# daac-tools/daachorse

Hardware: AMD Instinct MI355X
Metric: haystack GB/s scanned (find_overlapping_iter(..).count(), 100k-pattern bytewise automaton) (higher is better)
Workload: dtype u8/u32 integer

## Files before the change

### daachorse_amd/_build.py

```python
import os
import shutil
import subprocess

_HERE = os.path.dirname(os.path.abspath(__file__))
CSRC = os.path.join(_HERE, "csrc")
LIB_DIR = os.path.join(_HERE, "lib")
LIB_PATH = os.path.join(LIB_DIR, "libdaachorse_amd.so")

SOURCES = ["pma.cpp", "repack.cpp", "gram.cpp", "gram2.cpp", "gram4.cpp", "gram2w.cpp", "pfx.cpp", "builder.cpp", "charwise.cpp", "charwise_builder.cpp", "api_upload.hip", "api_scan.hip", "api_select.hip", "api_iter.hip", "api_options.hip", "scan_kernels.hip",
           "gram_kernels.hip", "gram2_kernels.hip", "gram4_kernels.hip", "pfx_kernels.hip", "emit3_kernels.hip", "find3_kernels.hip", "left3_kernels.hip", "gram2w_kernels.hip", "restart_kernels.hip", "charwise_kernels.hip", "synth.hip",
           "api_batch.hip", "batch_kernels.hip", "batch_hist_kernels.hip", "api_hist.hip", "hist_kernels.hip", "api_replace.hip", "replace_kernels.hip", "api_tokenize.hip", "tokenize_kernels.hip", "api_unigram.hip", "unigram_kernels.hip", "api_bpe.hip", "bpe_kernels.hip", "api_split.hip", "split_kernels.hip", "api_wordpiece.hip", "wordpiece_kernels.hip", "api_normalize.hip", "normalize_kernels.hip"]
HEADERS = ["api_internal.hpp", "pma.hpp", "repack.hpp", "gram.hpp", "gram2.hpp", "gram4.hpp", "gram4_filter.hpp", "gram4_index.hpp", "gram4_mph.hpp", "gram2w.hpp", "pfx.hpp", "charwise.hpp", "build_common.hpp", "device_tables.hpp", "chain_scan.hpp", "scan_engines.hpp", "restart_tables.hpp", "char_tables.hpp", "batch.hpp", "hist.hpp", "replace.hpp", "tokenize.hpp", "unigram.hpp", "bpe.hpp", "split.hpp", "wordpiece.hpp", "normalize.hpp",
           os.path.join("..", "..", "include", "daachorse_amd.h"),
           os.path.join("..", "..", "include", "daac_synth.h")]


def _hipcc():
    for cand in (shutil.which("hipcc"), "/opt/rocm/bin/hipcc"):
        if cand and os.path.exists(cand):
            return cand
    raise RuntimeError("hipcc not found: the HIP extension cannot be built")


def source_hash():
    import hashlib
    h = hashlib.sha256()
    for f in SOURCES + HEADERS:
        path = os.path.join(CSRC, f)
        h.update(os.path.basename(f).encode() + b"\0")
        with open(path, "rb") as fh:
            h.update(fh.read())
    return h.hexdigest()


def needs_build():
    if not os.path.exists(LIB_PATH):
        return True
    t = os.path.getmtime(LIB_PATH)
    files = [os.path.join(CSRC, f) for f in SOURCES + HEADERS]
    return any(os.path.exists(f) and os.path.getmtime(f) > t for f in files)


def build(force=False, verbose=False):
    if not force and not needs_build():
        return LIB_PATH
# ... 27 lines not shown
```

### daachorse_amd/csrc/api_internal.hpp

```cpp
#pragma once
#include <hip/hip_runtime.h>

#include <algorithm>
#include <atomic>
#include <cassert>
#include <cstdlib>
#include <chrono>
#include <cstring>
#include <map>
#include <memory>
#include <condition_variable>
#include <deque>
#include <functional>
#include <mutex>
#include <string>
#include <thread>
#include <utility>
#include <vector>

#include "charwise.hpp"
#include "device_tables.hpp"
#include "gram.hpp"
#include "gram2.hpp"
#include "gram4.hpp"
#include "gram2w.hpp"
#include "pfx.hpp"
#include "pma.hpp"
#include "repack.hpp"

namespace daac {
const char *last_error_cstr();

#define DAAC_OPTIONS(X)                                                                                                                      \
    X(seg_bytes, 0, 0)                                                                                                         \
    X(lds_budget, 96 * 1024, 1)                                                                                                              \
    X(dense_depth, -1, 1)                                                                                                                    \
    X(rows_share_pct, 45, 1)                                                                                                                 \
    X(blocks_per_cu, 0, 0)                                                                                                     \
    X(threads, 1024, 0)                                                                                                                      \
    X(iter_window, 64ll << 20, 0)                  \
    X(max_result_bytes, 8ll << 30, 0)                                                                                                        \
    X(gram_lds_budget, 158 * 1024, 1)                                                                                                        \
    X(gram_region, 0, 0)                                          \
    X(gram_slab, 4096, 0)                                                                                                                    \
    X(gram_ppl, 0, 0)                                                                      \
    X(gram_dense, -1, 0)                                                                                      \
    X(gram_rank_in_lds, -1, 1)                                                                                \
    X(gram_version, 0, 0)                   \
    X(gram4_arith, 1, 0)                  \
    X(gram4_filter, 1, 0)                      \
    X(gram4_mph, 8, 1)                    \
    X(gram2_dpp, 1, 0)                                                  \
    X(find3, 1, 0)                                                                                         \
    X(pfx_probe, 16384, 0)                                                             \
    X(pfx, 1, 1)                                 \
    X(gram_tail, -1, 0)                         \
    X(gram2_rfull, 1, 0)                                                            \
    X(emit, 1, 0)                            \
    X(emit_rec_per_kib, 32, 0)                               \
    X(restart_bpc, 8, 0)                                                              \
    X(restart_chain, 1, 0)                      \
    X(chain_rounds, 24, 0)                                                                                                                   \
    X(overlap_micro, 1, 0)                \
    X(pool, 1, 0)                                                                 \
    X(pool_keep, 0, 0)                                                                    \
    X(left3, 1, 0)                        \
    X(select_emit, 1, 0)                                   \
    X(find3_window, 1ll << 30, 0)                                \
    X(workspace_keep, 8ll << 30, 0)                          \
    X(char_map_lds, 1, 1)                                         \
    X(char_row_lds, 1, 1)                                                                      \
    X(batch_piece, 4096, 0)                                              \
    X(batch_lane_max, 16384, 0)           \
    X(hist_lds_bins, 16384, 0)            \
    X(batch_hist_wave_max, 2048, 0)                  \
    X(batch_hist_sort_max, 16384, 0)      \
    X(bpe_doc_max, 4096, 0)
// ... 387 lines not shown
```

### daachorse_amd/csrc/api_scan.hip

```cpp
#include "api_internal.hpp"

static daac_status scan_count_impl(daac_pma *pma, int mode, int engine, const uint8_t *hay, size_t len, size_t begin, int hay_is_device,
                                   void *stream_, uint64_t *count, uint64_t *checksum, uint64_t *result_dev, bool want_checksum);

namespace {

__global__ void repack8_kernel(const uint4 *in, uint2 *out, unsigned long long n, unsigned long long base, uint32_t end_bits) {
    for (unsigned long long i = static_cast<unsigned long long>(blockIdx.x) * blockDim.x + threadIdx.x; i < n; i += static_cast<unsigned long long>(gridDim.x) * blockDim.x) {
        const uint4 t = in[i];
        const unsigned long long end = (static_cast<unsigned long long>(t.y) << 32) | t.x;
        out[i] = uint2{t.w, static_cast<uint32_t>(end - base) | (t.z << end_bits)};
    }
}
__global__ void repack16_kernel(const daac_match *in, uint4 *out, unsigned long long n) {
    for (unsigned long long i = static_cast<unsigned long long>(blockIdx.x) * blockDim.x + threadIdx.x; i < n; i += static_cast<unsigned long long>(gridDim.x) * blockDim.x) {
        const daac_match m = in[i];
        out[i] = uint4{static_cast<uint32_t>(m.end), static_cast<uint32_t>(m.end >> 32), static_cast<uint32_t>(m.end - m.start), m.value};
    }
}

__global__ void shard_subtract_kernel(unsigned long long *r, const unsigned long long *h, unsigned long long from32) {
    r[0] -= h[0];
    r[1] -= h[1];
    r[2] -= h[2];
    r[2] += (r[1] & 0xffffffffull) * from32;
}

__global__ void shard_fixup_kernel(unsigned long long *r, unsigned long long begin32, unsigned long long c, unsigned long long s1,
                                   unsigned long long s2) {
    r[2] += (r[1] & 0xffffffffull) * begin32 + s2;
    r[1] += s1;
    r[0] += c;
}
// ... 341 lines not shown
        if (!want_checksum && t->gram4_ok && (gv == 4 || gv == 0 || (gv == 2 && !t->gram2.exact_ok)) && gram4_shape(t, cp)) {
            cp.kernel = CountKernel::gram4; cp.threads = cp.g4.threads; cp.lds_bytes = cp.g4.lds_bytes; cp.wq_entry = sizeof(uint4);
            return cp;
        }
        if (gv == 4 && !want_checksum)
            return refuse("gram_version = 4: the gram4 tables are not there for this automaton (or do not fit the LDS with the launch shape asked for)", CountKernel::gram4);
        if (!t->gram2.exact_ok) return refuse("GRAM second table set: `.count()` runs on the gram4 kernel (gram_version 0 or 4); the count + checksum kernel needs tables this dictionary has no room for", CountKernel::gram2);
        cp.kernel = CountKernel::gram2; cp.lds_bytes = gram2_lds_bytes(t->gram2, want_checksum);
    } else if (gram && g1_can) {
        cp.kernel = CountKernel::gram; cp.lds_bytes = t->gram.lds_bytes; cp.ppl = !t->gram.has_short && OPT(gram_ppl) != 16 ? 32 : 16;
        cp.n_deep = t->gram.n_deep; cp.C = t->gram.C; cp.K = t->gram.K;
    } else if (gram) {
        cp.kernel = CountKernel::gram2w; cp.threads = 1024; cp.lds_bytes = want_checksum ? t->gramw.lds_exact : t->gramw.lds_count;
        cp.n_deep = t->gramw.n_deep; cp.C = t->gramw.C; cp.K = 2;
    } else if (pfx) {
        cp.kernel = CountKernel::pfx; cp.region[0] = 65536; cp.region[1] = 262144;
        cp.threads = t->pfx.threads; cp.lds_bytes = t->pfx.lds_bytes; cp.wq_entry = sizeof(uint4);
    } else {
        cp.charwise = pma->charwise; cp.tier = on_tier(pma, t, mode, engine);
    }
    return cp;
}

std::pair<int, int> count_ids(const DeviceTables *t, const CountPlan &cp) {
    switch (cp.kernel) {
    case CountKernel::gram4: return {DAAC_ENGINE_GRAM, DAAC_KERNEL_GRAM_COUNT};
    case CountKernel::gram: case CountKernel::gram2: return {DAAC_ENGINE_GRAM, DAAC_KERNEL_GRAM_EXACT};
    case CountKernel::gram2w: return {DAAC_ENGINE_GRAM, DAAC_KERNEL_GRAM_WIDE};
    case CountKernel::pfx: return {DAAC_ENGINE_PFX, DAAC_KERNEL_PFX};
    default: return {cp.tier ? DAAC_ENGINE_TIERED : DAAC_ENGINE_DARRAY, micro_walker(t, cp.charwise, cp.tier) ? DAAC_KERNEL_MICRO : DAAC_KERNEL_SEGMENT};
    }
}

static std::string count_kernel_name(const CountPlan &cp) {
    static const char *const family[] = {"gram4", "gram", "gram2", "gram2w", "pfx"};
    if (cp.kernel == CountKernel::walkers) return cp.charwise ? "charwise" : cp.tier ? "tiered" : "darray";
    if (cp.kernel != CountKernel::gram4) return family[static_cast<int>(cp.kernel)];
    return "gram4 ppl=" + std::to_string(cp.ppl) + " dir=" + std::to_string(cp.g4.dir) + " waves=" + std::to_string(cp.g4.threads / 64) + " arith=" +
           std::to_string(cp.g4.arith) + " filter=" + std::to_string(cp.g4.filter) + " mph=" + std::to_string(cp.g4.mph) + " tail=" + (OPT(gram_tail) < 0 ? std::string("auto") : std::to_string(OPT(gram_tail) > 0 ? 1 : 0));
}

}
}

extern "C" {

static daac_status scan_count_impl(daac_pma *pma, int mode, int engine, const uint8_t *hay, size_t len, size_t begin, int hay_is_device,
                                   void *stream_, uint64_t *count, uint64_t *checksum, uint64_t *result_dev, bool want_checksum) {
    PmaScope scope_(pma);
    if (!pma || (len && !hay) || (!result_dev && (!count || (want_checksum && !checksum))) || begin > len) {
        set_error("bad argument");
        return DAAC_ERR_INVALID_ARGUMENT;
    }
    hipStream_t stream = static_cast<hipStream_t>(stream_);
    DeviceTables *t = nullptr;
    dbg_mark("count: entry");
    daac_status st = check_mode_kind(pma, mode);
    if (st != DAAC_OK) return st;
    if ((st = get_tables(pma, &t)) != DAAC_OK) return st;
    CountPlan cp = resolve_count(pma, t, mode, engine, want_checksum, len - begin);
    if (cp.probe && hay_is_device && !result_dev && len - begin >= (32ull << 20) && t->pfx_probe_word) {
        unsigned int *pin = pinned_words();
        unsigned int got = 0;
        unsigned int *tmp = const_cast<unsigned int *>(t->pfx_probe_word);
        HIP_TRY(launch_pfx_probe(t->pfx, hay + begin, len - begin, tmp, stream));
        HIP_TRY(hipMemcpyAsync(pin ? pin : &got, tmp, 4, hipMemcpyDeviceToHost, stream));
        HIP_TRY(hipStreamSynchronize(stream));
        if (pin) got = *pin;
        t->pfx_dense.store(got > static_cast<unsigned int>(std::max<int64_t>(0, OPT(pfx_probe))) ? 1 : 0);
        cp = resolve_count(pma, t, mode, engine, want_checksum, len - begin);
    }
    if (cp.st != DAAC_OK) { set_error(cp.err); return cp.st; }
    Plan pl;
    bool heads = false;
    if ((st = make_plan(pma, t, mode, cp.kernel != CountKernel::walkers ? DAAC_ENGINE_AUTO : engine, begin, len, pl, heads)) != DAAC_OK) return st;
    if (pl.a.nseg == 0 && begin == 0) pl.a.nseg = 1;
    void *staged = nullptr;
    const uint8_t *dev_hay = hay;
    if (!hay_is_device && len) {
        const uint64_t from = begin > pl.a.halo ? begin - pl.a.halo : 0;
        if ((st = stage_window(hay, from, len, stream, &staged, &dev_hay)) != DAAC_OK) return st;
    }
    std::unique_ptr<void, void (*)(void *)> g1(staged, [](void *p) { if (p) (void)hipFree(p); });
    pl.a.hay = dev_hay;
    unsigned long long *d_res = reinterpret_cast<unsigned long long *>(result_dev);
    DevBuf own;
    if (!d_res) { HIP_TRY(own.alloc(3 * sizeof(unsigned long long), stream)); d_res = static_cast<unsigned long long *>(own.p); }
    pl.a.result = d_res;
    bool find3_served = false;
    unsigned long long find3_sums[3] = {0, 0, 0};
    dbg_mark("count: plan made");
    if (!pma->charwise && engine == DAAC_ENGINE_AUTO && !pma->root_has_output() && len != begin &&
        ((mode == DAAC_FIND && pma->host.is_standard()) || (mode == DAAC_LEFTMOST_FIND && !pma->host.is_standard()))) {
        if ((st = find_count3(pma, t, dev_hay, begin, len, stream, d_res, want_checksum, mode == DAAC_LEFTMOST_FIND, find3_sums, &find3_served)) != DAAC_OK) return st;
    }
    dbg_mark("count: find3 back");
    ChainBuffers chain_buffers;
    if (!find3_served && pl.a.nseg != 0 && (st = chain_resolve(pma, t, pl, stream, chain_buffers)) != DAAC_OK) return st;
    if (!find3_served) HIP_TRY(hipMemsetAsync(d_res, 0, 3 * sizeof(unsigned long long), stream));
    void *flagbuf = nullptr;
    if (pl.leftmost && pma->root_has_output()) {
        HIP_TRY(hipMalloc(&flagbuf, sizeof(unsigned long long)));
        HIP_TRY(hipMemsetAsync(flagbuf, 0, sizeof(unsigned long long), stream));
        pl.a.flags = static_cast<unsigned long long *>(flagbuf);
    }
    std::unique_ptr<void, void (*)(void *)> g3(flagbuf, [](void *p) { if (p) (void)hipFree(p); });
    if (!find3_served) g_last_engine = count_ids(t, cp).first;
    g_last_kernel = find3_served ? "find3" : count_kernel_name(cp);
    if (find3_served) {
    } else if (cp.kernel != CountKernel::walkers && len != begin) {
        const uint64_t from = begin - std::min<uint64_t>(begin, pl.a.halo);
        const uint8_t *sub = dev_hay + from;
        GramArgs ga{};
        ga.lead = static_cast<uint32_t>(reinterpret_cast<uintptr_t>(sub) & 15u);
        ga.hay_al = sub - ga.lead;
        ga.vlen = ga.lead + static_cast<uint64_t>(len - from);
        uint64_t region = 2048;
        const int64_t region_opt = OPT(gram_region) > 0 ? OPT(gram_region) : static_cast<int64_t>(cp.region[(len - from) >= (1ull << 31)]);
        while (region * 2 <= static_cast<uint64_t>(std::max<int64_t>(2048, region_opt)) && region < (1ull << 30)) region *= 2;
        assert((region & (region - 1)) == 0 && region <= (1ull << 30));
        ga.ppl = cp.ppl;
        ga.region_bytes = region;
        ga.nregions = (ga.vlen + region - 1) / region;
        ga.result = d_res;
        const uint32_t threads = cp.threads, wpb = threads / 64;
        uint32_t bpc = static_cast<uint32_t>(OPT(blocks_per_cu));
        if (bpc == 0) bpc = std::max(1u, std::min(2048u / threads, (160u * 1024u) / cp.lds_bytes));
        const uint32_t blocks = static_cast<uint32_t>(
            std::max<uint64_t>(1, std::min<uint64_t>(static_cast<uint64_t>(t->num_cu) * bpc, (ga.nregions + wpb - 1) / wpb)));
        ga.wq_slab = static_cast<uint32_t>(std::max<int64_t>(64 * ga.ppl + 128 + 64, OPT(gram_slab)));
        ga.dense = OPT(gram_dense) >= 0 ? OPT(gram_dense) != 0 : cp.n_deep * 100 > cp.C * cp.C * cp.C * (cp.K == 3 ? cp.C : 1);
        const int64_t tail_opt = OPT(gram_tail);
        void *wq = nullptr;
        HIP_TRY(dev_malloc(&wq, static_cast<size_t>(blocks) * wpb * ga.wq_slab * cp.wq_entry, stream));
        ga.wq = static_cast<uint2 *>(wq);
        ga.sel_want = tail_opt < 0 ? ((len - begin) >= (1ull << 20) ? 2u : 0u) : tail_opt > 0 ? 1u : 0u;
        auto launch_count = [&](const GramArgs &g, uint32_t nblocks) -> hipError_t {
            switch (cp.kernel) {
            case CountKernel::gram4: return launch_gram4_scan(t->gram4, g, cp.g4, nblocks, stream);
            case CountKernel::gram: return launch_gram_scan(t->gram, g, nblocks, threads, stream);
            case CountKernel::gram2: return launch_gram2_scan(t->gram2, g, want_checksum, nblocks, threads, stream);
            case CountKernel::gram2w: return launch_gram2w_scan(t->gramw, g, want_checksum, nblocks, stream);
            case CountKernel::pfx: return launch_pfx_scan(t->pfx, g, want_checksum, nblocks, stream);
            default: return hipErrorInvalidValue;
            }
        };
        hipError_t le = launch_count(ga, blocks);
        DevBuf halo_res;
        if (le == hipSuccess && from != begin) {
            le = halo_res.alloc(3 * sizeof(unsigned long long), stream);
            if (le == hipSuccess) le = hipMemsetAsync(halo_res.p, 0, 3 * sizeof(unsigned long long), stream);
            GramArgs gh = ga;
            gh.vlen = ga.lead + (begin - from);
            gh.nregions = (gh.vlen + gh.region_bytes - 1) / gh.region_bytes;
            gh.result = static_cast<unsigned long long *>(halo_res.p);
            gh.sel_want = 0;
            if (le == hipSuccess) le = launch_count(gh, 1);
            if (le == hipSuccess) {
                hipLaunchKernelGGL(shard_subtract_kernel, dim3(1), dim3(1), 0, stream, d_res, static_cast<const unsigned long long *>(halo_res.p),
                                   static_cast<unsigned long long>(from & 0xffffffffull));
                le = hipGetLastError();
            }
        } else if (le == hipSuccess && from != 0) {
            hipLaunchKernelGGL(shard_fixup_kernel, dim3(1), dim3(1), 0, stream, d_res, static_cast<unsigned long long>(from & 0xffffffffull), 0ull, 0ull, 0ull);
            le = hipGetLastError();
        }
        dev_free(wq, stream);
        HIP_TRY(le);
    } else if (pl.a.nseg != 0) {
        HIP_TRY(launch(t, pl, 0, heads, stream));
    }
    unsigned long long flagv = 0;
    if (flagbuf) HIP_TRY(hipMemcpyAsync(&flagv, flagbuf, sizeof(flagv), hipMemcpyDeviceToHost, stream));
    if (result_dev && !count) {
        if (staged || flagbuf) HIP_TRY(hipStreamSynchronize(stream));
        return (flagv & 1ull) ? diverged() : DAAC_OK;
    }
    unsigned long long r[3];
    if (find3_served) {
        std::memcpy(r, find3_sums, sizeof(r));
    } else {
        HIP_TRY(hipMemcpyAsync(r, d_res, sizeof(r), hipMemcpyDeviceToHost, stream));
        HIP_TRY(hipStreamSynchronize(stream));
    }
    dbg_mark("count: result read");
    if (flagv & 1ull) return diverged();
    if (count) *count = r[0];
// ... 276 lines not shown
```

### daachorse_amd/csrc/device_tables.hpp

```cpp
#pragma once

#include <hip/hip_runtime.h>

#include <cstdint>

#include "../../include/daachorse_amd.h"
#include "gram4_mph.hpp"

namespace daac {

struct TierDev {
    const void *rows;
    const uint32_t *bcmap;
    const uint32_t *bfail;
    const uint2 *ssum;
    const uint8_t *cls;
    const uint4 *grec;
    const uint32_t *sopos;
    const uint32_t *outputs;
    const uint32_t *ohash;
    uint32_t C, NA, NB, N;
    uint32_t off_bcmap, off_bfail, off_ssum, off_cls, lds_bytes;
    uint32_t row32, root_flag;
};
// ... 56 lines not shown
};

struct GramDev {
    const uint32_t *cls32;
    const uint16_t *cid;
    const uint2 *combo;
    const uint32_t *bbits;
    const uint8_t *brank;
    const uint32_t *bsuper;
    const uint4 *drec;
    const uint2 *dhit;
    const uint4 *dhit4;
    const uint32_t *cfirst;
    uint32_t off_cid, off_combo, off_bbits, off_brank, off_bsuper, off_scratch, lds_bytes;
    uint32_t K, C, CC, CCC;
    uint32_t level_start, unused_byte, has_short;
    uint32_t rank_in_lds;
    uint32_t n_deep;
};

struct GramArgs {
    const uint8_t *hay_al;
    uint32_t lead;
    uint64_t vlen;
    uint64_t region_bytes;
    uint64_t nregions;
    unsigned long long *result;
    uint2 *wq;
    uint32_t wq_slab;
    uint32_t ppl;
    uint32_t dense;
    const uint32_t *sel;
    uint32_t sel_want;
};

hipError_t launch_gram_scan(const GramDev &dev, const GramArgs &a, uint32_t blocks, uint32_t threads, hipStream_t stream);

constexpr uint32_t kGram2OffH = 512;
struct Gram2Dev {
    const uint8_t *cls;
    const uint32_t *m;
    const void *sdir;
    const uint16_t *rfull;
    const uint16_t *cid4;
    const uint32_t *hsum;
    const uint4 *drec;
    const uint2 *dhit;
    const uint4 *dhit4;
    const uint32_t *cfirst;
    uint32_t m_bytes, s_bytes, cid_bytes, h_bytes;
    uint32_t off_m_count, off_s_count, off_ring_count, lds_count;
    uint32_t rfull_bytes, off_ring_rfull, lds_rfull, rfull_ok;
    uint32_t off_m_exact, off_s_exact, off_cid, off_ring_exact, lds_exact;
    uint32_t K, C, s16, unused_byte, n_deep, exact_ok;
    uint32_t xlane_dpp;
};
uint32_t gram2_lds_bytes(const Gram2Dev &dev, bool exact);

struct Gram2WDev {
    const uint8_t *cls;
    const unsigned long long *m;
    const uint32_t *sdir;
    const uint16_t *cid4;
    const uint32_t *hsum;
    const uint4 *drec;
    const uint4 *dhit;
// ... 211 lines not shown
```

### daachorse_amd/csrc/gram4_kernels.hip

```cpp
#include <hip/hip_runtime.h>

#include <algorithm>
#include <cstdint>
#include <utility>

#include "device_tables.hpp"
#include "gram4_filter.hpp"
#include "gram4_index.hpp"

namespace daac {

namespace {

typedef uint32_t g4_u32x4_t __attribute__((ext_vector_type(4)));
constexpr uint32_t kList4 = 256;
constexpr int kPass4Q2 = 2, kPass4Q1 = 1;
constexpr uint32_t kProbePercent4 = 3;
typedef __attribute__((address_space(3))) const uint32_t lds4_cu32;
typedef __attribute__((address_space(3))) uint32_t lds4_u32;
typedef __attribute__((address_space(3))) const uint16_t lds4_cu16;
typedef __attribute__((address_space(3))) uint16_t lds4_u16;
typedef __attribute__((address_space(3))) const uint8_t lds4_cu8;
typedef __attribute__((address_space(3))) g4_u32x4_t lds4_u32x4;

__device__ __forceinline__ uint32_t pin4(uint32_t x) {
    asm("" : "+v"(x));
    return x;
}
__device__ __forceinline__ uint32_t mad24(uint32_t a, uint32_t b, uint32_t c) {
    uint32_t d;
    asm("v_mad_u32_u24 %0, %1, %2, %3" : "=v"(d) : "v"(a), "s"(b), "v"(c));
    return d;
}
__device__ __forceinline__ uint32_t wave_shr1_4(uint32_t v, uint32_t lane0) {
    uint32_t d = lane0;
    asm volatile("s_nop 1\nv_mov_b32_dpp %0, %1 wave_shr:1 row_mask:0xf bank_mask:0xf" : "+v"(d) : "v"(v));
    return d;
}
__device__ __forceinline__ uint32_t g4_wave_scan(uint32_t v) {
    v += static_cast<uint32_t>(__builtin_amdgcn_update_dpp(0, static_cast<int>(v), 0x111, 0xf, 0xf, false));
    v += static_cast<uint32_t>(__builtin_amdgcn_update_dpp(0, static_cast<int>(v), 0x112, 0xf, 0xf, false));
    v += static_cast<uint32_t>(__builtin_amdgcn_update_dpp(0, static_cast<int>(v), 0x114, 0xf, 0xf, false));
    v += static_cast<uint32_t>(__builtin_amdgcn_update_dpp(0, static_cast<int>(v), 0x118, 0xf, 0xf, false));
    v += static_cast<uint32_t>(__builtin_amdgcn_update_dpp(0, static_cast<int>(v), 0x142, 0xa, 0xf, false));
    v += static_cast<uint32_t>(__builtin_amdgcn_update_dpp(0, static_cast<int>(v), 0x143, 0xc, 0xf, false));
    return v;
}
template <typename F, int... I>
__device__ __forceinline__ void g4_turns(F &&f, std::integer_sequence<int, I...>) {
    (void)(... && f(std::integral_constant<int, I>{}));
}
template <int N, typename F>
__device__ __forceinline__ void g4_upto(uint32_t n, F &&f) {
    if constexpr (N > 1) {
        if (n < static_cast<uint32_t>(N)) {
            g4_upto<N - 1>(n, f);
            return;
        }
    }
    f(std::integral_constant<int, N>{});
}
__device__ __forceinline__ unsigned long long g4_wave_sum(unsigned long long v) {
#pragma unroll
    for (int off = 32; off > 0; off >>= 1) v += __shfl_down(v, off, 64);
    return v;
}
__device__ __forceinline__ void g4_copy(void *dst, const void *src, uint32_t bytes) {
    const uint4 *s = reinterpret_cast<const uint4 *>(src);
    uint4 *d = reinterpret_cast<uint4 *>(dst);
    for (uint32_t i = threadIdx.x; i < bytes / 16; i += blockDim.x) d[i] = s[i];
}
__device__ __forceinline__ void g4_reduce(unsigned long long cnt, unsigned long long *scratch, unsigned long long *result) {
    const unsigned long long c = g4_wave_sum(cnt);
    __syncthreads();
    const int wave = threadIdx.x >> 6, lane = threadIdx.x & 63;
    if (lane == 0) scratch[wave] = c;
    __syncthreads();
    if (threadIdx.x == 0) {
        unsigned long long r0 = 0;
        for (int w = 0; w < static_cast<int>((blockDim.x + 63) >> 6); ++w) r0 += scratch[w];
        if (r0) atomicAdd(result, r0);
    }
}

}

template <int K, int Q, bool ARITH, int DIR, bool TAIL, bool FILT, bool MPH = false>
__device__ __forceinline__ void gram4_body(const Gram4Dev &g, const GramArgs &a, const Gram4Lds &L, char *smem) {
    static_assert(!(FILT && TAIL), "the filter runs in front of the plain records");
    static_assert(!(FILT && DIR == 0), "the filter's Bloom array lies where the per-word directory would");
    static_assert(!MPH || FILT, "the perfect hash serves the survivors of the filter");
    constexpr int P = 16 * Q;
    constexpr int GS = 8;
    constexpr int PB = !FILT ? 1 : Q == 2 ? kPass4Q2 : kPass4Q1;
    constexpr uint32_t SB = 64u * P;
    constexpr uint32_t SLOT = SB + 32u;
    const uint32_t offM = L.off_m, offS = L.off_s, offC = L.off_cls;
    const uint32_t lo = g.lo, OTH = g.C - 1u, C = g.C;
    auto cls_of = [&](uint32_t byte) -> uint32_t {
        if (ARITH) {
            const uint32_t u = byte - lo;
            return u < OTH ? u : OTH;
        }
        return *reinterpret_cast<lds4_cu8 *>(static_cast<uintptr_t>(offC + byte));
    };
    auto lds_u32 = [&](uint32_t addr) -> uint32_t { return *reinterpret_cast<lds4_cu32 *>(static_cast<uintptr_t>(addr)); };
    auto below = [&](uint32_t k) -> uint32_t { return (1u << k) - 1u; };

    const uint32_t lane = threadIdx.x & 63;
    const uint32_t lane_off = pin4(lane * (16u * Q));
    const uint32_t wave_in_wg = __builtin_amdgcn_readfirstlane(threadIdx.x >> 6);
    const uint32_t C4 = C * 4u, CC4 = C * C * 4u;
    const uint32_t offM1 = g4i_off1(offM, C);
    const uint32_t ub4 = g.unused_byte * 0x01010101u;
    const uint8_t *__restrict__ hay = a.hay_al;
    const uint64_t nwaves = static_cast<uint64_t>(gridDim.x) * (blockDim.x >> 6);
    const uint32_t tb = L.off_wave + wave_in_wg * L.wave_stride;
    const uint32_t listb = wave_in_wg * (kList4 * 2u);
    const uint64_t slab_index = (static_cast<uint64_t>(blockIdx.x) * (blockDim.x >> 6) + wave_in_wg) * a.wq_slab;
    uint4 *__restrict__ slab4 = reinterpret_cast<uint4 *>(a.wq) + slab_index;
    uint32_t wq_n = 0, slab_hi = 0;
    uint64_t epoch_base = 0;
    const uint32_t drain_early = wave_in_wg * 64u;

    unsigned long long tot_cnt = 0;
    uint32_t cnt32 = 0;

    auto load_chunk = [&](uint64_t v) -> uint4 {
        if (v >= a.vlen) return uint4{ub4, ub4, ub4, ub4};
        const g4_u32x4_t q = __builtin_nontemporal_load(reinterpret_cast<const g4_u32x4_t *>(hay + v));
        uint4 r{q.x, q.y, q.z, q.w};
        if (v < a.lead || v + 16 > a.vlen) {
            uint32_t w[4] = {r.x, r.y, r.z, r.w};
            for (int b = 0; b < 16; ++b) {
                const uint64_t p = v + b;
                if (p < a.lead || p >= a.vlen) w[b >> 2] = (w[b >> 2] & ~(0xffu << (8 * (b & 3)))) | (g.unused_byte << (8 * (b & 3)));
            }
            r = uint4{w[0], w[1], w[2], w[3]};
        }
        return r;
    };
    auto raw_at = [&](uint64_t p) -> uint32_t { return (p >= a.lead && p < a.vlen) ? hay[p] : g.unused_byte; };
    auto read_ahead = [&](uint64_t v) -> unsigned long long {
        unsigned long long x;
        if (v >= a.lead && v + 8 <= a.vlen) {
            __builtin_memcpy(&x, hay + v, 8);
        } else {
            x = 0;
            for (int b = 7; b >= 0; --b) x = (x << 8) | ((v + b >= a.lead && v + b < a.vlen) ? hay[v + b] : g.unused_byte);
        }
        return x;
    };
    auto tail_count = [&](const uint4 &rr, unsigned long long text) -> uint32_t {
        const uint32_t edges = rr.x & 15u;
        const unsigned long long path = (static_cast<unsigned long long>(rr.w) << 32) | rr.z;
        const unsigned long long diff = path ^ text;
        uint32_t same = diff ? static_cast<uint32_t>(__builtin_ctzll(diff)) >> 3 : 8u;
        same = same < edges ? same : edges;
        return __popc((rr.x >> 4) & ((2u << same) - 1u) & 0x1ffu);
    };
    auto drain = [&]() {
        const uint4 *__restrict__ recs = TAIL ? g.drec_t : g.drec_c;
        uint32_t n_in = wq_n;
        bool raw = !TAIL;
        while (n_in != 0) {
            uint32_t n_out = 0;
            for (uint32_t base = 0; base < n_in; base += 64u) {
                const uint32_t i = base + lane;
                const bool live = i < n_in;
                uint4 e = uint4{0u, 0u, 0u, 0u};
                if (live) e = slab4[i];
                uint32_t state, n_ahead, pos = e.x;
                unsigned long long ah;
                if (raw) {
// ... 314 lines not shown
        }
#pragma unroll
        for (int b = 0; b < NB; ++b)
            if (pm[b] != 0) {
                const uint32_t s = static_cast<uint32_t>(__popcll(pm[b]));
                const bool full = sb_n + s >= 64u;
                unsigned long long mine;
                asm("s_bfm_b64 %0, %1, %2" : "=s"(mine) : "s"(s), "s"(sb_n));
                sb_n += s;
                if (full) {
                    consume_pending();
                    const unsigned long long upper = ~0ull << (sb_n - s);
                    uint32_t lo64;
                    asm("v_cndmask_b32_e64 %0, %1, %2, %3" : "=v"(fp_pos) : "v"(sb_pos), "v"(r_pos[b]), "s"(upper));
                    asm("v_cndmask_b32_e64 %0, %1, %2, %3" : "=v"(lo64) : "v"(sb_lo), "v"(r_lo[b]), "s"(upper));
                    asm("v_cndmask_b32_e64 %0, %1, %2, %3" : "=v"(fp_t0) : "v"(sb_t0), "v"(r_t0[b]), "s"(upper));
                    if constexpr (MPH) hash_and_ask(lo64); else rank_and_ask(lo64);
                    pend_valid = true;
                    sb_n -= 64u;
                    asm("s_bfm_b64 %0, %1, 0" : "=s"(mine) : "s"(sb_n));
                }
                asm("v_cndmask_b32_e64 %0, %0, %1, %2" : "+v"(sb_pos) : "v"(r_pos[b]), "s"(mine));
                asm("v_cndmask_b32_e64 %0, %0, %1, %2" : "+v"(sb_lo) : "v"(r_lo[b]), "s"(mine));
                asm("v_cndmask_b32_e64 %0, %0, %1, %2" : "+v"(sb_t0) : "v"(r_t0[b]), "s"(mine));
            }
    };
    auto process_full = [&]() {
        while (st_n + q_tail - q_head >= 64u) {
            if constexpr (FILT && PB > 1) g4_upto<PB>((st_n + q_tail - q_head) >> 6, process_pass);
            else process_batch(64u);
        }
    };

    uint64_t region = static_cast<uint64_t>(blockIdx.x) * (blockDim.x >> 6) + wave_in_wg;
    while (region < a.nregions) {
      slab_hi = static_cast<uint32_t>((region * a.region_bytes) >> 31);
      epoch_base = static_cast<uint64_t>(slab_hi) << 31;
      for (; region < a.nregions && static_cast<uint32_t>((region * a.region_bytes) >> 31) == slab_hi; region += nwaves) {
        const uint64_t rbase = region * a.region_bytes;
        const uint64_t rend = rbase + a.region_bytes < a.vlen ? rbase + a.region_bytes : a.vlen;
        uint32_t carry = 0, tail4 = 0;
#pragma unroll
        for (int i = 0; i < K; ++i) carry |= (rbase >= static_cast<uint64_t>(K - i) ? cls_of(raw_at(rbase - (K - i))) : OTH) << (8 * i);
#pragma unroll
        for (int i = 0; i < 4; ++i) tail4 |= (rbase >= static_cast<uint64_t>(4 - i) ? raw_at(rbase - (4 - i)) : static_cast<uint32_t>(g.unused_byte)) << (8 * i);
        tail4 = __builtin_amdgcn_readfirstlane(tail4);
        carry = __builtin_amdgcn_readfirstlane(carry);
        uint32_t mcarry;
        {
            uint32_t x = (((carry >> (8 * (K - 1))) & 0xffu) << 2) + offM;
            x += __umul24((carry >> (8 * (K - 2))) & 0xffu, C4);
            if (K == 3) x += __umul24(carry & 0xffu, CC4);
            mcarry = __builtin_amdgcn_readfirstlane(lds_u32(x));
        }

        const uint32_t rlen = static_cast<uint32_t>(rend - rbase);
        const uint32_t fast_lo = rbase < 16u ? SB : 0u;
        const uint32_t fast_hi = rlen & ~(SB - 1u);
        auto fetch = [&](uint32_t off, uint4 (&out)[Q]) {
            if (off >= fast_lo && off < fast_hi) {
                const uint8_t *__restrict__ base = hay + rbase + off;
                uint32_t voff = lane_off;
                asm volatile("" : "+v"(voff));
#pragma unroll
                for (int q = 0; q < Q; ++q) {
                    const g4_u32x4_t t = __builtin_nontemporal_load(reinterpret_cast<const g4_u32x4_t *>(base + voff + 16u * q));
                    out[q] = uint4{t.x, t.y, t.z, t.w};
                }
                return;
            }
            const uint64_t s0 = rbase + off;
#pragma unroll
            for (int q = 0; q < Q; ++q) out[q] = uint4{ub4, ub4, ub4, ub4};
            if (off < rlen) {
#pragma unroll
                for (int q = 0; q < Q; ++q) out[q] = load_chunk(s0 + lane * P + 16u * q);
            } else if (lane == 0 && off < rlen + SB) {
                out[0] = load_chunk(s0);
            }
        };
        uint4 pf0[Q], pf1[Q];
        fetch(0u, pf0);
        fetch(SB, pf1);
        const uint32_t rbias = static_cast<uint32_t>(rbase - epoch_base) - (tb + 16u - 3u);

        for (uint32_t off = 0; off < rlen; off += SB) {
            if (wq_n + 64u * P + 128u + drain_early > a.wq_slab) drain();
            uint4 cur[Q];
#pragma unroll
            for (int q = 0; q < Q; ++q) { cur[q] = pf0[q]; pf0[q] = pf1[q]; }
            consume_pending();
            __builtin_amdgcn_s_setprio(0);
            fetch(off + 2u * SB, pf1);

            if (q_tail != q_head) {
                const uint32_t n_left = q_tail - q_head;
                derive(st_n, n_left);
                st_n += n_left;
            }
            q_head = q_tail = 0;
            const uint32_t slot = tb;
            const uint32_t my_text = slot + 16u + lane * P;
            posbias = rbias + off;
#pragma unroll
            for (int q = 0; q < Q; ++q)
                *reinterpret_cast<lds4_u32x4 *>(static_cast<uintptr_t>(my_text + 16u * q)) = g4_u32x4_t{cur[q].x, cur[q].y, cur[q].z, cur[q].w};
            if (lane == 0) {
                *reinterpret_cast<lds4_u32 *>(static_cast<uintptr_t>(slot + 12u)) = tail4;
                *reinterpret_cast<lds4_u32x4 *>(static_cast<uintptr_t>(slot + 16u + SB)) = g4_u32x4_t{pf0[0].x, pf0[0].y, pf0[0].z, pf0[0].w};
            }
            tail4 = __builtin_amdgcn_readlane(cur[Q - 1].w, 63);

            uint32_t kx[K + P];
#pragma unroll
            for (int q = 0; q < Q; ++q) {
                const uint32_t w[4] = {cur[q].x, cur[q].y, cur[q].z, cur[q].w};
// ... 58 lines not shown
                if (__ballot(H != 0u) == 0) break;
                const uint32_t n = __popc(H);
                const uint32_t incl = g4_wave_scan(n);
                const uint32_t tot = __builtin_amdgcn_readlane(incl, 63);
                const uint32_t first = q_tail + incl - n;
                const uint32_t room = first < kList4 ? kList4 - first : 0u;
                const uint32_t lim = n < room ? n : room;
                const uint32_t at = pin4(listb + (first << 1));
                g4_turns([&](auto tc) -> bool {
                    constexpr uint32_t t = decltype(tc)::value;
                    const bool w = t < lim;
                    if (__ballot(w) == 0) return false;
                    if (w) {
                        *reinterpret_cast<lds4_u16 *>(static_cast<uintptr_t>(at + 2u * t)) = static_cast<uint16_t>(text_adj + __builtin_ctz(H));
                        H &= H - 1u;
                    }
                    return true;
                }, std::make_integer_sequence<int, P>{});
                const uint32_t in = std::min(tot, kList4 - q_tail);
                q_tail += in;
                process_full();
                if (in == tot) break;
                const uint32_t n_left = q_tail - q_head;
                if (lane < n_left) {
                    const uint16_t v = *reinterpret_cast<lds4_cu16 *>(static_cast<uintptr_t>(listb + ((q_head + lane) << 1)));
                    *reinterpret_cast<lds4_u16 *>(static_cast<uintptr_t>(listb + (lane << 1))) = v;
                }
                q_head = 0;
                q_tail = n_left;
            }
        }
        tot_cnt += cnt32;
        cnt32 = 0;
      }
      if (st_n + q_tail - q_head != 0) process_batch(st_n + q_tail - q_head);
      if (FILT && sb_n != 0) { survivors_ask(sb_n); sb_n = 0; }
      consume_pending();
      finish_second();
      drain();
      tot_cnt += cnt32;
      cnt32 = 0;
    }
    g4_reduce(tot_cnt, reinterpret_cast<unsigned long long *>(smem), a.result);
}

template <int K, int Q, bool ARITH, int DIR, int TPB, bool FILT, bool MPH = false>
__global__ __launch_bounds__(TPB) void gram4_kernel(const Gram4Dev g, const GramArgs a, const Gram4Lds L) {
    extern __shared__ __attribute__((aligned(16))) char smem[];
    constexpr int DIRC = DIR == 0 ? 1 : DIR;
    if (!ARITH) g4_copy(smem + L.off_cls, g.cls, 256);
    g4_copy(smem + L.off_m, g.m, g.m_bytes);
    uint32_t *votes = reinterpret_cast<uint32_t *>(smem + L.off_wave);
    if (threadIdx.x == 0) *votes = 0;
    __syncthreads();
    if (__builtin_amdgcn_groupstaticsize() != 0) __builtin_trap();
    bool tail = a.sel_want == 1u;
    if (a.sel_want == 2u) {
        const uint64_t span = a.vlen > a.lead + 16 ? a.vlen - a.lead - 8 : 0;
        bool go = false;
        if (span != 0) {
            unsigned long long h = (static_cast<unsigned long long>(threadIdx.x) + 1) * 0x9E3779B97F4A7C15ull;
            h ^= h >> 29;
            const uint64_t p = a.lead + 3 + (h % (span - 3));
            const uint8_t *t = a.hay_al + p;
            const uint32_t OTH = g.C - 1u;
            auto cl = [&](uint32_t b) -> uint32_t {
                if (ARITH) { const uint32_t u = b - g.lo; return u < OTH ? u : OTH; }
                return reinterpret_cast<const uint8_t *>(smem + L.off_cls)[b];
            };
            const uint32_t *m = reinterpret_cast<const uint32_t *>(smem + L.off_m);
            const uint32_t c0 = cl(t[-3]), c1 = cl(t[-2]), c2 = cl(t[-1]), d = cl(t[0]), k1 = cl(t[1]);
            const uint32_t ctx = K == 3 ? (c0 * g.C + c1) * g.C + c2 : c1 * g.C + c2;
            const uint32_t w = m[ctx];
            if ((w >> d) & 1u & (d < OTH ? 1u : 0u)) {
                uint32_t rank = __popc(w & ((1u << d) - 1u));
                for (uint32_t j = ctx & ~3u; j < ctx; ++j) rank += __popc(m[j] & 0x3fffffffu);
// ... 98 lines not shown
```

Baseline: 1834.

## Add tapered small-region tail with atomic dynamic claiming in gram4 scan

Measured after the change: 1883, median of 6. 1.03x the previous value.

```diff
diff --git a/daachorse_amd/_build.py b/daachorse_amd/_build.py
--- a/daachorse_amd/_build.py
+++ b/daachorse_amd/_build.py
@@ -10,7 +10,7 @@
 SOURCES = ["pma.cpp", "repack.cpp", "gram.cpp", "gram2.cpp", "gram4.cpp", "gram2w.cpp", "pfx.cpp", "builder.cpp", "charwise.cpp", "charwise_builder.cpp", "api_upload.hip", "api_scan.hip", "api_select.hip", "api_iter.hip", "api_options.hip", "scan_kernels.hip",
            "gram_kernels.hip", "gram2_kernels.hip", "gram4_kernels.hip", "pfx_kernels.hip", "emit3_kernels.hip", "find3_kernels.hip", "left3_kernels.hip", "gram2w_kernels.hip", "restart_kernels.hip", "charwise_kernels.hip", "synth.hip",
            "api_batch.hip", "batch_kernels.hip", "batch_hist_kernels.hip", "api_hist.hip", "hist_kernels.hip", "api_replace.hip", "replace_kernels.hip", "api_tokenize.hip", "tokenize_kernels.hip", "api_unigram.hip", "unigram_kernels.hip", "api_bpe.hip", "bpe_kernels.hip", "api_split.hip", "split_kernels.hip", "api_wordpiece.hip", "wordpiece_kernels.hip", "api_normalize.hip", "normalize_kernels.hip"]
-HEADERS = ["api_internal.hpp", "pma.hpp", "repack.hpp", "gram.hpp", "gram2.hpp", "gram4.hpp", "gram4_filter.hpp", "gram4_index.hpp", "gram4_mph.hpp", "gram2w.hpp", "pfx.hpp", "charwise.hpp", "build_common.hpp", "device_tables.hpp", "chain_scan.hpp", "scan_engines.hpp", "restart_tables.hpp", "char_tables.hpp", "batch.hpp", "hist.hpp", "replace.hpp", "tokenize.hpp", "unigram.hpp", "bpe.hpp", "split.hpp", "wordpiece.hpp", "normalize.hpp",
+HEADERS = ["api_internal.hpp", "pma.hpp", "repack.hpp", "gram.hpp", "gram2.hpp", "gram4.hpp", "gram4_claims.hpp", "gram4_filter.hpp", "gram4_index.hpp", "gram4_mph.hpp", "gram2w.hpp", "pfx.hpp", "charwise.hpp", "build_common.hpp", "device_tables.hpp", "chain_scan.hpp", "scan_engines.hpp", "restart_tables.hpp", "char_tables.hpp", "batch.hpp", "hist.hpp", "replace.hpp", "tokenize.hpp", "unigram.hpp", "bpe.hpp", "split.hpp", "wordpiece.hpp", "normalize.hpp",
            os.path.join("..", "..", "include", "daachorse_amd.h"),
            os.path.join("..", "..", "include", "daac_synth.h")]
 
diff --git a/daachorse_amd/csrc/api_internal.hpp b/daachorse_amd/csrc/api_internal.hpp
--- a/daachorse_amd/csrc/api_internal.hpp
+++ b/daachorse_amd/csrc/api_internal.hpp
@@ -43,6 +43,8 @@
     X(gram_lds_budget, 158 * 1024, 1)                                                                                                        \
     X(gram_region, 0, 0)                                          \
     X(gram_slab, 4096, 0)                                                                                                                    \
+    X(gram_region_small, 0, 0)            \
+    X(gram_taper_split, -1, 0)            \
     X(gram_ppl, 0, 0)                                                                      \
     X(gram_dense, -1, 0)                                                                                      \
     X(gram_rank_in_lds, -1, 1)                                                                                \
diff --git a/daachorse_amd/csrc/api_scan.hip b/daachorse_amd/csrc/api_scan.hip
--- a/daachorse_amd/csrc/api_scan.hip
+++ b/daachorse_amd/csrc/api_scan.hip
@@ -1,4 +1,8 @@
 #include "api_internal.hpp"
+#include "gram4_claims.hpp"
+
+static constexpr int64_t kTaperSmall = 32768;
+static constexpr uint64_t kTaperPerWave = 2;
 
 static daac_status scan_count_impl(daac_pma *pma, int mode, int engine, const uint8_t *hay, size_t len, size_t begin, int hay_is_device,
                                    void *stream_, uint64_t *count, uint64_t *checksum, uint64_t *result_dev, bool want_checksum);
@@ -406,12 +410,12 @@
     }
 }
 
-static std::string count_kernel_name(const CountPlan &cp) {
+static std::string count_kernel_name(const CountPlan &cp, const std::string &regions = std::string()) {
     static const char *const family[] = {"gram4", "gram", "gram2", "gram2w", "pfx"};
     if (cp.kernel == CountKernel::walkers) return cp.charwise ? "charwise" : cp.tier ? "tiered" : "darray";
     if (cp.kernel != CountKernel::gram4) return family[static_cast<int>(cp.kernel)];
     return "gram4 ppl=" + std::to_string(cp.ppl) + " dir=" + std::to_string(cp.g4.dir) + " waves=" + std::to_string(cp.g4.threads / 64) + " arith=" +
-           std::to_string(cp.g4.arith) + " filter=" + std::to_string(cp.g4.filter) + " mph=" + std::to_string(cp.g4.mph) + " tail=" + (OPT(gram_tail) < 0 ? std::string("auto") : std::to_string(OPT(gram_tail) > 0 ? 1 : 0));
+           std::to_string(cp.g4.arith) + " filter=" + std::to_string(cp.g4.filter) + " mph=" + std::to_string(cp.g4.mph) + regions + " tail=" + (OPT(gram_tail) < 0 ? std::string("auto") : std::to_string(OPT(gram_tail) > 0 ? 1 : 0));
 }
 
 }
@@ -471,7 +475,8 @@
     dbg_mark("count: find3 back");
     ChainBuffers chain_buffers;
     if (!find3_served && pl.a.nseg != 0 && (st = chain_resolve(pma, t, pl, stream, chain_buffers)) != DAAC_OK) return st;
-    if (!find3_served) HIP_TRY(hipMemsetAsync(d_res, 0, 3 * sizeof(unsigned long long), stream));
+    const bool g4_launch = cp.kernel == CountKernel::gram4 && len != begin;
+    if (!find3_served && !g4_launch) HIP_TRY(hipMemsetAsync(d_res, 0, 3 * sizeof(unsigned long long), stream));
     void *flagbuf = nullptr;
     if (pl.leftmost && pma->root_has_output()) {
         HIP_TRY(hipMalloc(&flagbuf, sizeof(unsigned long long)));
@@ -495,19 +500,50 @@
         assert((region & (region - 1)) == 0 && region <= (1ull << 30));
         ga.ppl = cp.ppl;
         ga.region_bytes = region;
-        ga.nregions = (ga.vlen + region - 1) / region;
         ga.result = d_res;
         const uint32_t threads = cp.threads, wpb = threads / 64;
         uint32_t bpc = static_cast<uint32_t>(OPT(blocks_per_cu));
         if (bpc == 0) bpc = std::max(1u, std::min(2048u / threads, (160u * 1024u) / cp.lds_bytes));
+        uint64_t small = region, split = ~0ull;
+        if (g4_launch) {
+            const uint64_t full_waves = static_cast<uint64_t>(t->num_cu) * bpc * wpb;
+            small = 2048;
+            const int64_t small_opt = OPT(gram_region_small) > 0 ? OPT(gram_region_small) : kTaperSmall;
+            while (small * 2 <= static_cast<uint64_t>(small_opt) && small * 2 <= region) small *= 2;
+            if (OPT(gram_taper_split) >= 0) {
+                split = static_cast<uint64_t>(OPT(gram_taper_split));
+            } else if (small < region) {
+                const uint64_t tail = full_waves * kTaperPerWave * small;
+                if (ga.vlen > tail && (ga.vlen - tail) / region >= 2 * full_waves) split = ga.vlen - tail;
+            }
+        }
+        const G4Taper taper = g4_taper_plan(ga.vlen, region, small, split);
+        ga.region_small = taper.small;
+        ga.nlarge = taper.nlarge;
+        ga.nregions = taper.nregions;
         const uint32_t blocks = static_cast<uint32_t>(
             std::max<uint64_t>(1, std::min<uint64_t>(static_cast<uint64_t>(t->num_cu) * bpc, (ga.nregions + wpb - 1) / wpb)));
         ga.wq_slab = static_cast<uint32_t>(std::max<int64_t>(64 * ga.ppl + 128 + 64, OPT(gram_slab)));
+        ga.static_rounds = ga.nlarge == ga.nregions ? ~0u : static_cast<uint32_t>(std::max<uint64_t>(1, ga.nlarge / (static_cast<uint64_t>(blocks) * wpb)));
+        if (g4_launch) {
+            if (ga.nregions + static_cast<uint64_t>(blocks) * wpb >= (1ull << 32)) {
+                set_error("gram4: more regions than 32-bit claims hold (gram_region / gram_region_small too small for this haystack)");
+                return DAAC_ERR_UNSUPPORTED;
+            }
+            const uint64_t owned = ga.static_rounds == ~0u ? ga.nregions : std::min<uint64_t>(ga.nregions, static_cast<uint64_t>(ga.static_rounds) * blocks * wpb);
+            g_last_kernel = count_kernel_name(cp, " regions=" + std::to_string(ga.nregions) + " claims=" + std::to_string(ga.nregions - owned));
+        }
         ga.dense = OPT(gram_dense) >= 0 ? OPT(gram_dense) != 0 : cp.n_deep * 100 > cp.C * cp.C * cp.C * (cp.K == 3 ? cp.C : 1);
         const int64_t tail_opt = OPT(gram_tail);
+        constexpr size_t kWqHead = 256;
         void *wq = nullptr;
-        HIP_TRY(dev_malloc(&wq, static_cast<size_t>(blocks) * wpb * ga.wq_slab * cp.wq_entry, stream));
-        ga.wq = static_cast<uint2 *>(wq);
+        HIP_TRY(dev_malloc(&wq, kWqHead + static_cast<size_t>(blocks) * wpb * ga.wq_slab * cp.wq_entry, stream));
+        ga.wq = reinterpret_cast<uint2 *>(static_cast<char *>(wq) + kWqHead);
+        ga.claim = static_cast<unsigned long long *>(wq);
+        if (g4_launch) {
+            const hipError_t ce = hipMemsetAsync(wq, 0, 128, stream);
+            if (ce != hipSuccess) { dev_free(wq, stream); HIP_TRY(ce); }
+        }
         ga.sel_want = tail_opt < 0 ? ((len - begin) >= (1ull << 20) ? 2u : 0u) : tail_opt > 0 ? 1u : 0u;
         auto launch_count = [&](const GramArgs &g, uint32_t nblocks) -> hipError_t {
             switch (cp.kernel) {
@@ -523,10 +559,13 @@
         DevBuf halo_res;
         if (le == hipSuccess && from != begin) {
             le = halo_res.alloc(3 * sizeof(unsigned long long), stream);
-            if (le == hipSuccess) le = hipMemsetAsync(halo_res.p, 0, 3 * sizeof(unsigned long long), stream);
+            if (le == hipSuccess && !g4_launch) le = hipMemsetAsync(halo_res.p, 0, 3 * sizeof(unsigned long long), stream);
             GramArgs gh = ga;
             gh.vlen = ga.lead + (begin - from);
             gh.nregions = (gh.vlen + gh.region_bytes - 1) / gh.region_bytes;
+            gh.nlarge = gh.nregions;
+            gh.static_rounds = ~0u;
+            gh.claim = ga.claim + 8;
             gh.result = static_cast<unsigned long long *>(halo_res.p);
             gh.sel_want = 0;
             if (le == hipSuccess) le = launch_count(gh, 1);
diff --git a/daachorse_amd/csrc/device_tables.hpp b/daachorse_amd/csrc/device_tables.hpp
--- a/daachorse_amd/csrc/device_tables.hpp
+++ b/daachorse_amd/csrc/device_tables.hpp
@@ -112,6 +112,10 @@
     uint32_t dense;
     const uint32_t *sel;
     uint32_t sel_want;
+    uint64_t region_small;
+    uint64_t nlarge;
+    unsigned long long *claim;
+    uint32_t static_rounds;
 };
 
 hipError_t launch_gram_scan(const GramDev &dev, const GramArgs &a, uint32_t blocks, uint32_t threads, hipStream_t stream);
diff --git a/daachorse_amd/csrc/gram4_claims.hpp b/daachorse_amd/csrc/gram4_claims.hpp
--- /dev/null
+++ b/daachorse_amd/csrc/gram4_claims.hpp
@@ -0,0 +1,44 @@
+#pragma once
+#include <cstdint>
+
+#if defined(__HIPCC__) || defined(__CUDACC__)
+#define G4C_HD __host__ __device__ __forceinline__
+#else
+#define G4C_HD inline
+#endif
+
+namespace daac {
+
+struct G4Taper {
+    uint64_t large = 0, small = 0;
+    uint64_t nlarge = 0;
+    uint64_t nregions = 0;
+};
+struct G4Region {
+    uint64_t base;
+    uint64_t size;
+};
+
+inline G4Taper g4_taper_plan(uint64_t vlen, uint64_t large, uint64_t small, uint64_t split) {
+    G4Taper t;
+    t.large = large;
+    t.small = small < large ? small : large;
+    const uint64_t all_large = (vlen + large - 1) / large;
+    t.nlarge = split / large < all_large ? split / large : all_large;
+    const uint64_t behind = t.nlarge * large < vlen ? vlen - t.nlarge * large : 0;
+    t.nregions = t.nlarge + (behind + t.small - 1) / t.small;
+    return t;
+}
+
+G4C_HD uint32_t g4_log2(uint64_t pow2) {
+    uint32_t l = 0;
+    while ((1ull << l) < pow2) ++l;
+    return l;
+}
+G4C_HD G4Region g4_claim_region(uint64_t claim, uint32_t large_log2, uint32_t small_log2, uint64_t nlarge) {
+    if (claim < nlarge) return G4Region{claim << large_log2, 1ull << large_log2};
+    return G4Region{(nlarge << large_log2) + ((claim - nlarge) << small_log2), 1ull << small_log2};
+}
+G4C_HD G4Region g4_claim_region(uint64_t claim, const G4Taper &t) { return g4_claim_region(claim, g4_log2(t.large), g4_log2(t.small), t.nlarge); }
+
+}
diff --git a/daachorse_amd/csrc/gram4_kernels.hip b/daachorse_amd/csrc/gram4_kernels.hip
--- a/daachorse_amd/csrc/gram4_kernels.hip
+++ b/daachorse_amd/csrc/gram4_kernels.hip
@@ -5,6 +5,7 @@
 #include <utility>
 
 #include "device_tables.hpp"
+#include "gram4_claims.hpp"
 #include "gram4_filter.hpp"
 #include "gram4_index.hpp"
 
@@ -68,9 +69,15 @@
 __device__ __forceinline__ void g4_copy(void *dst, const void *src, uint32_t bytes) {
     const uint4 *s = reinterpret_cast<const uint4 *>(src);
     uint4 *d = reinterpret_cast<uint4 *>(dst);
-    for (uint32_t i = threadIdx.x; i < bytes / 16; i += blockDim.x) d[i] = s[i];
-}
-__device__ __forceinline__ void g4_reduce(unsigned long long cnt, unsigned long long *scratch, unsigned long long *result) {
+    const uint32_t n = bytes / 16, bd = blockDim.x;
+    uint32_t i = threadIdx.x;
+    for (; i + 3u * bd < n; i += 4u * bd) {
+        const uint4 v0 = s[i], v1 = s[i + bd], v2 = s[i + 2u * bd], v3 = s[i + 3u * bd];
+        d[i] = v0; d[i + bd] = v1; d[i + 2u * bd] = v2; d[i + 3u * bd] = v3;
+    }
+    for (; i < n; i += bd) d[i] = s[i];
+}
+__device__ __forceinline__ void g4_reduce(unsigned long long cnt, unsigned long long *scratch, unsigned long long *claim, unsigned long long *result) {
     const unsigned long long c = g4_wave_sum(cnt);
     __syncthreads();
     const int wave = threadIdx.x >> 6, lane = threadIdx.x & 63;
@@ -79,7 +86,52 @@
     if (threadIdx.x == 0) {
         unsigned long long r0 = 0;
         for (int w = 0; w < static_cast<int>((blockDim.x + 63) >> 6); ++w) r0 += scratch[w];
-        if (r0) atomicAdd(result, r0);
+        if (r0) atomicAdd(claim + 1, r0);
+        __threadfence();
+        if (atomicAdd(claim + 2, 1ull) + 1ull == gridDim.x) {
+            __threadfence();
+            result[0] = atomicAdd(claim + 1, 0ull);
+            result[1] = 0;
+            result[2] = 0;
+        }
+    }
+}
+__device__ __forceinline__ uint4 g4_load_chunk(const GramArgs &a, uint32_t unused_byte, uint64_t v) {
+    const uint32_t ub4 = unused_byte * 0x01010101u;
+    if (v >= a.vlen) return uint4{ub4, ub4, ub4, ub4};
+    const g4_u32x4_t q = __builtin_nontemporal_load(reinterpret_cast<const g4_u32x4_t *>(a.hay_al + v));
+    uint4 r{q.x, q.y, q.z, q.w};
+    if (v < a.lead || v + 16 > a.vlen) {
+        uint32_t w[4] = {r.x, r.y, r.z, r.w};
+        for (int b = 0; b < 16; ++b) {
+            const uint64_t p = v + b;
+            if (p < a.lead || p >= a.vlen) w[b >> 2] = (w[b >> 2] & ~(0xffu << (8 * (b & 3)))) | (unused_byte << (8 * (b & 3)));
+        }
+        r = uint4{w[0], w[1], w[2], w[3]};
+    }
+    return r;
+}
+template <int Q>
+__device__ __forceinline__ void g4_fetch_ahead(const GramArgs &a, uint32_t unused_byte, uint64_t rbase, uint32_t rlen, uint32_t off, uint4 (&out)[Q]) {
+    constexpr uint32_t P = 16u * Q, SB = 64u * P;
+    const uint32_t lane = threadIdx.x & 63, ub4 = unused_byte * 0x01010101u;
+    const uint32_t fast_lo = rbase < 16u ? SB : 0u, fast_hi = rlen & ~(SB - 1u);
+    if (off >= fast_lo && off < fast_hi) {
+        const uint8_t *__restrict__ base = a.hay_al + rbase + off;
+#pragma unroll
+        for (int q = 0; q < Q; ++q) {
+            const g4_u32x4_t t = __builtin_nontemporal_load(reinterpret_cast<const g4_u32x4_t *>(base + lane * P + 16u * q));
+            out[q] = uint4{t.x, t.y, t.z, t.w};
+        }
+        return;
+    }
+#pragma unroll
+    for (int q = 0; q < Q; ++q) out[q] = uint4{ub4, ub4, ub4, ub4};
+    if (off < rlen) {
+#pragma unroll
+        for (int q = 0; q < Q; ++q) out[q] = g4_load_chunk(a, unused_byte, rbase + off + lane * P + 16u * q);
+    } else if (lane == 0 && off < rlen + SB) {
+        out[0] = g4_load_chunk(a, unused_byte, rbase + off);
     }
 }
 
@@ -126,20 +178,7 @@
     unsigned long long tot_cnt = 0;
     uint32_t cnt32 = 0;
 
-    auto load_chunk = [&](uint64_t v) -> uint4 {
-        if (v >= a.vlen) return uint4{ub4, ub4, ub4, ub4};
-        const g4_u32x4_t q = __builtin_nontemporal_load(reinterpret_cast<const g4_u32x4_t *>(hay + v));
-        uint4 r{q.x, q.y, q.z, q.w};
-        if (v < a.lead || v + 16 > a.vlen) {
-            uint32_t w[4] = {r.x, r.y, r.z, r.w};
-            for (int b = 0; b < 16; ++b) {
-                const uint64_t p = v + b;
-                if (p < a.lead || p >= a.vlen) w[b >> 2] = (w[b >> 2] & ~(0xffu << (8 * (b & 3)))) | (g.unused_byte << (8 * (b & 3)));
-            }
-            r = uint4{w[0], w[1], w[2], w[3]};
-        }
-        return r;
-    };
+    auto load_chunk = [&](uint64_t v) -> uint4 { return g4_load_chunk(a, g.unused_byte, v); };
     auto raw_at = [&](uint64_t p) -> uint32_t { return (p >= a.lead && p < a.vlen) ? hay[p] : g.unused_byte; };
     auto read_ahead = [&](uint64_t v) -> unsigned long long {
         unsigned long long x;
@@ -520,13 +559,33 @@
         }
     };
 
-    uint64_t region = static_cast<uint64_t>(blockIdx.x) * (blockDim.x >> 6) + wave_in_wg;
-    while (region < a.nregions) {
-      slab_hi = static_cast<uint32_t>((region * a.region_bytes) >> 31);
+    const uint32_t nregions = static_cast<uint32_t>(a.nregions), nlarge = static_cast<uint32_t>(a.nlarge), nwaves32 = static_cast<uint32_t>(nwaves);
+    const uint32_t lg_large = static_cast<uint32_t>(__builtin_ctzll(a.region_bytes)), lg_small = static_cast<uint32_t>(__builtin_ctzll(a.region_small));
+    const uint32_t claim_base = nwaves32 * a.static_rounds;
+    uint32_t static_left = a.static_rounds - 1u;
+    auto claim_next = [&]() -> uint32_t {
+        unsigned long long c = 0;
+        if (lane == 0) c = __hip_atomic_fetch_add(a.claim, 1ull, __ATOMIC_RELAXED, __HIP_MEMORY_SCOPE_AGENT);
+        return claim_base + __builtin_amdgcn_readfirstlane(static_cast<uint32_t>(c));
+    };
+    auto region_of = [&](uint32_t r) -> G4Region { return g4_claim_region(r, lg_large, lg_small, nlarge); };
+    uint32_t region = blockIdx.x * (blockDim.x >> 6) + wave_in_wg;
+    constexpr bool AHEAD = Q == 2 && TAIL;
+    uint4 pf0[Q], pf1[Q];
+    auto fetch_ahead = [&](uint32_t r) {
+        const G4Region rg = region_of(r);
+        const uint32_t len = static_cast<uint32_t>((rg.base + rg.size < a.vlen ? rg.base + rg.size : a.vlen) - rg.base);
+        g4_fetch_ahead<Q>(a, g.unused_byte, rg.base, len, 0u, pf0);
+        g4_fetch_ahead<Q>(a, g.unused_byte, rg.base, len, SB, pf1);
+    };
+    if constexpr (AHEAD) if (region < nregions) fetch_ahead(region);
+    while (region < nregions) {
+      slab_hi = static_cast<uint32_t>(region_of(region).base >> 31);
       epoch_base = static_cast<uint64_t>(slab_hi) << 31;
-      for (; region < a.nregions && static_cast<uint32_t>((region * a.region_bytes) >> 31) == slab_hi; region += nwaves) {
-        const uint64_t rbase = region * a.region_bytes;
-        const uint64_t rend = rbase + a.region_bytes < a.vlen ? rbase + a.region_bytes : a.vlen;
+      for (;;) {
+        const G4Region rg = region_of(region);
+        const uint64_t rbase = rg.base;
+        const uint64_t rend = rbase + rg.size < a.vlen ? rbase + rg.size : a.vlen;
         uint32_t carry = 0, tail4 = 0;
 #pragma unroll
         for (int i = 0; i < K; ++i) carry |= (rbase >= static_cast<uint64_t>(K - i) ? cls_of(raw_at(rbase - (K - i))) : OTH) << (8 * i);
@@ -567,9 +626,12 @@
                 out[0] = load_chunk(s0);
             }
         };
-        uint4 pf0[Q], pf1[Q];
-        fetch(0u, pf0);
-        fetch(SB, pf1);
+        if constexpr (!AHEAD) {
+            fetch(0u, pf0);
+            fetch(SB, pf1);
+        }
+        uint32_t region_next = region + nwaves32;
+        if (static_left != 0) --static_left; else region_next = claim_next();
         const uint32_t rbias = static_cast<uint32_t>(rbase - epoch_base) - (tb + 16u - 3u);
 
         for (uint32_t off = 0; off < rlen; off += SB) {
@@ -694,6 +756,9 @@
         }
         tot_cnt += cnt32;
         cnt32 = 0;
+        region = region_next;
+        if (!(region < nregions && static_cast<uint32_t>(region_of(region).base >> 31) == slab_hi)) break;
+        if constexpr (AHEAD) fetch_ahead(region);
       }
       if (st_n + q_tail - q_head != 0) process_batch(st_n + q_tail - q_head);
       if (FILT && sb_n != 0) { survivors_ask(sb_n); sb_n = 0; }
@@ -702,8 +767,9 @@
       drain();
       tot_cnt += cnt32;
       cnt32 = 0;
-    }
-    g4_reduce(tot_cnt, reinterpret_cast<unsigned long long *>(smem), a.result);
+      if constexpr (AHEAD) if (region < nregions) fetch_ahead(region);
+    }
+    g4_reduce(tot_cnt, reinterpret_cast<unsigned long long *>(smem), a.claim, a.result);
 }
 
 template <int K, int Q, bool ARITH, int DIR, int TPB, bool FILT, bool MPH = false>
```
